# decadenza/SimpleStereo

Hardware: AMD Instinct MI355X
Metric: disparity MPixels/s (H*W*nDisp per second) (higher is better)
Workload: dtype f32

## Files before the change

### simplestereo_amd/csrc/asw_pipe_kernel.hip.h

```cpp
#pragma once
#include "asw_kernels.hip.h"
#ifndef SSAMD_KERNEL_TU
#include "lab_kernels.hip.h"
#endif

#ifndef SSAMD_PIPE_SENTINEL
#define SSAMD_PIPE_SENTINEL 1
#endif

namespace ssamd {

#ifndef SSAMD_KERNEL_TU
static constexpr int TADV_COLS = 64;
template <bool BYTES>
__device__ __forceinline__ void asw_tad_tile(const void *__restrict__ srcL, const void *__restrict__ srcR, unsigned char *__restrict__ evol,
                                             int W, int pad, int minD, int Dc, int Se, int erow0, int erows, int evolW, int rd, long long npix_total,
                                             int bx, int by, int bz, char *smem)
{
    uint32_t *const sL = reinterpret_cast<uint32_t *>(smem);
    uint32_t *const sR = sL + TADV_COLS;
    const int r = erow0 + by, z = bz, uc0 = bx * TADV_COLS;
    const int P = Se >> 2, dlo = minD + z * Dc, dhi = dlo + Dc - 1;
    const int u0 = uc0 - pad, xr0 = u0 - dhi;
    auto pixel = [&](const void *src, int col) -> uint32_t {
        const size_t q = (size_t)r * W + col;
        if constexpr (BYTES) {
            typedef uint32_t __attribute__((aligned(1))) u32_unaligned;
            const uint8_t *const b = reinterpret_cast<const uint8_t *>(src) + 3 * q;
            return (long long)q + 1 < npix_total ? (*reinterpret_cast<const u32_unaligned *>(b) & 0xffffffu)
                                                 : ((uint32_t)b[0] | ((uint32_t)b[1] << 8) | ((uint32_t)b[2] << 16));
        } else {
            return reinterpret_cast<const PixRec *>(src)[q].bgrx;
        }
    };
    for (int k = threadIdx.x; k < 2 * TADV_COLS + Dc; k += blockDim.x) {
        const bool isL = k < TADV_COLS;
        const int col = isL ? u0 + k : xr0 + (k - TADV_COLS);
        const uint32_t v = (unsigned)col < (unsigned)W ? pixel(isL ? srcL : srcR, col) : 0x80000000u;
        (isL ? sL : sR)[isL ? k : k - TADV_COLS] = v;
    }
    __syncthreads();
    const int ncols = min(TADV_COLS, evolW - uc0);
    uint32_t *const out = reinterpret_cast<uint32_t *>(evol + (((size_t)z * erows + by) * (size_t)evolW + uc0) * Se);
    auto dword = [&](int c, int slot, uint32_t lp) {
        uint32_t v = 0;
        const int d0 = rd == 6 ? 6 * (slot >> 1) + 4 * (slot & 1) : 4 * slot, nv = rd == 6 && (slot & 1) ? 2 : 4;
        if (!(lp >> 31) && d0 < Dc) {
            const uint32_t *const rp = sR + c + (Dc - 1) - d0;
#pragma unroll
            for (int q = 0; q < 4; ++q) {
                const uint32_t rv = q < nv && d0 + q < Dc ? rp[-q] : 0x80000000u;
                if (!(rv >> 31)) v |= min(__builtin_amdgcn_sad_u8(lp, rv, 0u), 40u) << (8 * q);
            }
        }
        return v;
    };
    if ((P & 3) == 0) {
        const int P4 = P >> 2;
        uint4 *const out4 = reinterpret_cast<uint4 *>(out);
        for (int k = threadIdx.x; k < ncols * P4; k += blockDim.x) {
            const int c = k / P4, s4 = 4 * (k - c * P4);
            const uint32_t lp = sL[c];
            out4[k] = make_uint4(dword(c, s4, lp), dword(c, s4 + 1, lp), dword(c, s4 + 2, lp), dword(c, s4 + 3, lp));
        }
        return;
    }
    for (int k = threadIdx.x; k < ncols * P; k += blockDim.x) {
        const int c = k / P, slot = k - c * P;
        out[k] = dword(c, slot, sL[c]);
    }
}

__global__ __launch_bounds__(256) void asw_tad_volume_kernel(const PixRec *__restrict__ recL, const PixRec *__restrict__ recR,
                                                             unsigned char *__restrict__ evol, int W, int pad, int minD, int Dc,
                                                             int Se, int erow0, int erows, int evolW, int rd = 4)
{
    extern __shared__ __attribute__((aligned(16))) char smem[];
    asw_tad_tile<false>(recL, recR, evol, W, pad, minD, Dc, Se, erow0, erows, evolW, rd, 0, blockIdx.x, blockIdx.y, blockIdx.z, smem);
}

struct AswPrepassArgs {
    const uint8_t *bgrL, *bgrR;
    PixRec *recL, *recR;
    unsigned char *evol;
    long long npix_total;
    int W, pad, minD, Dc, Se, erow0, erows, evolW, rd;
    int lab_blocks, ex, ey;
};
__global__ __launch_bounds__(256) void asw_prepass_kernel(const AswPrepassArgs P)
{
    extern __shared__ __attribute__((aligned(16))) char smem[];
    if ((int)blockIdx.x < P.lab_blocks) {
        SSAMD_LAB_TABLES_IN_LDS(T)
        const long long np = (long long)P.erows * P.W, first = (long long)P.erow0 * P.W;
        const uint8_t *const bl = P.bgrL + 3 * first, *const br = P.bgrR + 3 * first;
        PixRec *const rl = P.recL + first, *const rr = P.recR + first;
        typedef uint32_t __attribute__((aligned(1))) u32_unaligned;
        for (long long q = (long long)blockIdx.x * blockDim.x + threadIdx.x; q < 2 * np; q += (long long)P.lab_blocks * blockDim.x) {
            const bool right = q >= np;
            const long long p = right ? q - np : q;
            const uint8_t *const bgr = right ? br : bl;
            uint32_t B, G, R;
            if (p + 1 < np) {
                const uint32_t v = *reinterpret_cast<const u32_unaligned *>(bgr + 3 * p);
                B = v & 0xff; G = (v >> 8) & 0xff; R = (v >> 16) & 0xff;
            } else {
                B = bgr[3 * p]; G = bgr[3 * p + 1]; R = bgr[3 * p + 2];
            }
            PixRec o;
            bgr_to_lab(B, G, R, o.L, o.a, o.b, T);
            o.bgrx = B | (G << 8) | (R << 16);
            (right ? rr : rl)[p] = o;
        }
        return;
    }
    const int b = (int)blockIdx.x - P.lab_blocks, bx = b % P.ex, by = (b / P.ex) % P.ey, bz = b / (P.ex * P.ey);
    asw_tad_tile<true>(P.bgrL, P.bgrR, P.evol, P.W, P.pad, P.minD, P.Dc, P.Se, P.erow0, P.erows, P.evolW, P.rd, P.npix_total, bx, by, bz, smem);
}

#endif

template <bool WITH_COSTS, int SLC = 0, int SRC = 0, int SEC = 0, bool CG = false>
__global__ __launch_bounds__(ASW_MAX_THREADS, 3) void asw_aggregate_pipe_kernel(const AswArgs A)
{
    constexpr bool STATIC = SLC > 0;
    static_assert(!CG || STATIC, "compile-time geometry belongs to a static tile");
    constexpr int RX = ASW_RX;
    constexpr int NWR = asw_nwr(RX);
    extern __shared__ __attribute__((aligned(16))) char smem[];
    constexpr AswGeom SG = asw_pipe_geom_constexpr(AswPipeTile<SLC, SRC, SEC>::id);
    static_assert(!STATIC || (SG.SL == SLC && SG.SR == SRC && SG.Se == SEC), "the strides name the tile");
    const AswGeom &g = CG ? SG : A.g;
    float *const wL = reinterpret_cast<float *>(smem + g.off_wL);
    float *const wR = reinterpret_cast<float *>(smem + g.off_wR);
    unsigned char *const eT0 = reinterpret_cast<unsigned char *>(smem + g.off_e);
    float4 *const labL = reinterpret_cast<float4 *>(smem + g.off_labL);
    float4 *const labR = reinterpret_cast<float4 *>(smem + g.off_labR);
    uint32_t *const bgrL = reinterpret_cast<uint32_t *>(smem + g.off_bgrL);
    uint32_t *const bgrR = reinterpret_cast<uint32_t *>(smem + g.off_bgrR);
    u64 *const bestL = reinterpret_cast<u64 *>(smem + g.off_bestL);
    u64 *const bestR = reinterpret_cast<u64 *>(smem + g.off_bestR);
    float4 *const cenLab = reinterpret_cast<float4 *>(smem + g.off_cen);
    float *const proxS = reinterpret_cast<float *>(smem + g.off_prox);

    const int tid = threadIdx.x, nthr = blockDim.x;
    const int W = A.W, win = CG ? AswPipeTile<SLC, SRC, SEC>::id.win : A.win, p = CG ? AswPipeTile<SLC, SRC, SEC>::id.win / 2 : A.pad;
    const int Tx = g.Tx, Dc = g.Dc, nL = g.nL, nR = g.nR, nRc = g.nRc, SR = g.SR, Se = g.Se;
    const int JC = g.JC, NC = g.NC;
    int bx = blockIdx.x;
    if ((gridDim.x & 7) == 0) bx = (bx & 7) * (gridDim.x >> 3) + (bx >> 3);
    const int x0 = bx * Tx;
    const int y = asw_out_row(A, blockIdx.y);
    const int dlo = A.minD + blockIdx.z * Dc;
    const int dhi = dlo + Dc - 1;
    if (min(x0 + Tx - 1, W - 1) - dlo < 0) {
        if (A.disp)
            for (int k = threadIdx.x; k < Tx && x0 + k < W; k += blockDim.x)
                A.disp[(size_t)(y - A.row0) * W + x0 + k] = (int16_t)(x0 + k);
        return;
    }
    const int segL_lo = x0 - p, xrc_lo = x0 - dhi, segR_lo = xrc_lo - p;
    const int phase = g.dephase ? __builtin_amdgcn_readfirstlane((int)(threadIdx.x >> 8)) : 1;

    float accN[RX][ASW_RD], accS[RX][ASW_RD];
#pragma unroll
    for (int a = 0; a < RX; ++a)
#pragma unroll
        for (int b = 0; b < ASW_RD; ++b) { accN[a][b] = 0.f; accS[a][b] = 0.f; }

    for (int k = tid; k < Tx; k += nthr) bestL[k] = KEY_NONE;
    for (int k = tid; k <= nRc; k += nthr) bestR[k] = KEY_NONE;
    for (int c = tid; c < Tx + nRc; c += nthr) {
        const bool isL = c < Tx;
        const int ccol = isL ? x0 + c : xrc_lo + (c - Tx);
        float4 v = make_float4(0.f, 0.f, 0.f, 0.f);
        if ((unsigned)ccol < (unsigned)W) {
            const PixRec q = (isL ? A.recL : A.recR)[(size_t)y * W + ccol];
            v = make_float4(q.L, q.a, q.b, 1.f);
        }
        cenLab[c] = v;
    }

    const int i_lo = max(0, p - y), i_hi = min(win, A.H + p - y);

    auto stage_row = [&](int i) {
        int tids = threadIdx.x;
        asm volatile("" : "+v"(tids));
        const int buf = i & 1, r = y - p + i;
        for (int k = tids; k < win; k += nthr) proxS[buf * win + k] = A.prox[i * win + k];
        const PixRec *const rowL = A.recL + (size_t)r * W;
        const PixRec *const rowR = A.recR + (size_t)r * W;
        for (int k = tids; k < nL + nR; k += nthr) {
            const bool isL = k < nL;
            const int idx = isL ? k : k - nL;
            const int col = (isL ? segL_lo : segR_lo) + idx;
            PixRec v;
            v.L = SSAMD_PIPE_SENTINEL ? __builtin_inff() : 0.f;
            v.a = v.b = 0.f;
            v.bgrx = 0u;
            if ((unsigned)col < (unsigned)W) v = (isL ? rowL : rowR)[col];
            (isL ? labL + buf * nL : labR + buf * nR)[idx] = make_float4(v.L, v.a, v.b, 0.f);
            if (!A.evol) (isL ? bgrL + buf * nL : bgrR + buf * nR)[idx] = v.bgrx;
        }
    };
    auto build_e = [&](int i, int t_lo, int t_hi) {
        int tidb = threadIdx.x;
        asm volatile("" : "+v"(tidb));
        unsigned char *const eT = eT0 + (i & 1) * g.e_bytes;
        const uint32_t *const bgrLc = bgrL + (i & 1) * nL, *const bgrRc = bgrR + (i & 1) * nR;
        const int e_q = nthr / nL, e_r = nthr - e_q * nL;
        int t = t_lo + tidb;
        int sp = t / nL, ul = t - sp * nL;
        while (t < t_hi) {
            const uint32_t lp = bgrLc[ul];
            const uint32_t *const rp = bgrRc + (ul + (Dc - 1) - 8 * sp);
            uint32_t lo = 0, hi = 0;
#pragma unroll
            for (int k = 0; k < 4; ++k) {
                lo |= min(__builtin_amdgcn_sad_u8(lp, rp[-k], 0u), 40u) << (8 * k);
                hi |= min(__builtin_amdgcn_sad_u8(lp, rp[-4 - k], 0u), 40u) << (8 * k);
            }
            uint32_t *const dst = reinterpret_cast<uint32_t *>(eT + ul * Se) + 2 * sp;
            dst[0] = lo;
            if (2 * sp + 1 < g.DG) dst[1] = hi;
            t += nthr; ul += e_r; sp += e_q;
            if (ul >= nL) { ul -= nL; ++sp; }
        }
    };
    auto load_e = [&](int i) {
        int tidd = threadIdx.x;
        asm volatile("" : "+v"(tidd));
        const int r = y - p + i;
        const unsigned char *const src = A.evol + (((size_t)blockIdx.z * A.erows + (r - A.erow0)) * (size_t)A.evolW + x0) * Se;
        unsigned char *const dst = eT0 + (i & 1) * g.e_bytes;
        const int bytes = nL * Se, lane16 = (tidd & 63) * 16;
        for (int k = __builtin_amdgcn_readfirstlane(tidd >> 6) * 1024; k < bytes; k += (nthr >> 6) * 1024)
            if (k + lane16 < bytes)
                __builtin_amdgcn_global_load_lds((const void *)(src + k + lane16),
                                                 (__attribute__((address_space(3))) void *)(dst + k), 16, 0, 0);
    };
    auto build_weights = [&](int i, int jb, int je, int rb) {
        int tidw = threadIdx.x;
        asm volatile("" : "+v"(tidw));
        const float4 *const labLc = labL + (i & 1) * nL, *const labRc = labR + (i & 1) * nR;
        const float *const prow = proxS + (i & 1) * win;
        const int ncen = Tx + nRc;
        const int full = ncen / nthr * nthr, rest = ncen - full;
        int slen = je - jb, nseg = 1;
        if (rest > 0 && full > 0) {
            slen = max(ASW_WB, (je - jb + nthr / rest - 1) / (nthr / rest));
            slen = (slen + ASW_WB - 1) / ASW_WB * ASW_WB;
            nseg = (je - jb + slen - 1) / slen;
        }
        const int ntasks = full + rest * nseg;
        for (int t = tidw; t < ntasks; t += nthr) {
            int c = t, jb_t = jb, je_t = je;
            if (t >= full && nseg > 1) {
                const int q = t - full, sgm = q / rest;
                c = full + q - sgm * rest;
                jb_t = jb + sgm * slen;
                je_t = min(je, jb_t + slen);
            }
            const bool isL = c < Tx;
            const int cc = isL ? c : c - Tx;
            const float4 cen = cenLab[c];
            const float4 *const seg = (isL ? labLc : labRc) + cc;
            const int stride = isL ? g.SL : SR;
            float *const wout = (isL ? wL : wR) + cc + (rb - jb) * stride;
            const int col0 = (isL ? x0 : xrc_lo) + cc - p;
            const uint32_t cmask = cen.w != 0.f ? 0xffffffffu : 0u;
            int j = jb_t;
            const float4 *sp = seg + j;
            const float *pp = prow + j;
            float *wp = wout + j * stride;
            int col = col0 + j;
            const int stride4 = ASW_WB * stride;
            for (; j + ASW_WB <= je_t; j += ASW_WB, sp += ASW_WB, pp += ASW_WB, wp += stride4, col += ASW_WB) {
                float4 tp[ASW_WB];
                float pr[ASW_WB], wv[ASW_WB];
#pragma unroll
                for (int u = 0; u < ASW_WB; ++u) { tp[u] = sp[u]; pr[u] = pp[u]; }
#pragma unroll
                for (int u = 0; u < ASW_WB; ++u) {
                    asm volatile("" ::"v"(tp[u].w));
                    const float dL = tp[u].x - cen.x, da = tp[u].y - cen.y, db = tp[u].z - cen.z;
                    wv[u] = fmaf(db, db, fmaf(da, da, dL * dL));
                }
#pragma unroll
                for (int u = 0; u < ASW_WB; ++u) wv[u] = __builtin_amdgcn_sqrtf(wv[u]);
#pragma unroll
                for (int u = 0; u < ASW_WB; ++u) wv[u] = asw_weight_finish(wv[u], A.kC, pr[u]);
#pragma unroll
                for (int u = 0; u < ASW_WB; ++u) {
                    if constexpr (SSAMD_PIPE_SENTINEL) {
                        wp[u * stride] = wv[u];
                    } else {
                        const uint32_t m = (unsigned)(col + u) < (unsigned)W ? cmask : 0u;
                        wp[u * stride] = __uint_as_float(__float_as_uint(wv[u]) & m);
                    }
                }
            }
            if (j < je_t) {
                float4 tp[ASW_WB];
                float pr[ASW_WB], wv[ASW_WB];
#pragma unroll
                for (int u = 0; u < ASW_WB; ++u) {
                    const int jj = min(j + u, je_t - 1);
                    tp[u] = seg[jj];
                    pr[u] = prow[jj];
                }
#pragma unroll
                for (int u = 0; u < ASW_WB; ++u) {
                    asm volatile("" ::"v"(tp[u].w));
                    const float dL = tp[u].x - cen.x, da = tp[u].y - cen.y, db = tp[u].z - cen.z;
                    wv[u] = fmaf(db, db, fmaf(da, da, dL * dL));
                }
#pragma unroll
                for (int u = 0; u < ASW_WB; ++u) wv[u] = __builtin_amdgcn_sqrtf(wv[u]);
#pragma unroll
                for (int u = 0; u < ASW_WB; ++u) wv[u] = asw_weight_finish(wv[u], A.kC, pr[u]);
#pragma unroll
                for (int u = 0; u < ASW_WB; ++u) {
                    const int jj = min(j + u, je_t - 1);
                    if constexpr (SSAMD_PIPE_SENTINEL) {
                        wout[jj * stride] = wv[u];
                    } else {
                        const uint32_t m = (unsigned)(col0 + jj) < (unsigned)W ? cmask : 0u;
                        wout[jj * stride] = __uint_as_float(__float_as_uint(wv[u]) & m);
                    }
                }
            }
        }
    };
    auto chunk_end = [&](int c) { return c == NC - 1 ? win : (c + 1) * JC; };
    const int nE = nL * ((g.DG + 1) >> 1);
    auto build_next = [&](int i, int c, int cb) {
        const bool more_rows = i + 1 < i_hi;
#ifdef SSAMD_PIPE_BUILD_PRIO
        __builtin_amdgcn_s_setprio(SSAMD_PIPE_BUILD_PRIO);
#endif
#ifndef SSAMD_ABLATE_STAGE
        if (c == 0 && more_rows) stage_row(i + 1);
#endif
        if (c == 0 && more_rows && A.evol) load_e(i + 1);
#ifndef SSAMD_ABLATE_WEIGHTS
        if (c + 1 < NC) build_weights(i, (c + 1) * JC, chunk_end(c + 1), (cb ^ 1) * g.JCmax);
        else if (more_rows) build_weights(i + 1, 0, chunk_end(0), (cb ^ 1) * g.JCmax);
#endif
#ifndef SSAMD_ABLATE_E
        if (c >= 1 && more_rows && !A.evol) build_e(i + 1, (int)((long long)nE * (c - 1) / (NC - 1)), (int)((long long)nE * c / (NC - 1)));
#endif
#ifdef SSAMD_PIPE_BUILD_PRIO
        __builtin_amdgcn_s_setprio(0);
#endif
    };

    stage_row(i_lo);
    if (A.evol) load_e(i_lo);
    __syncthreads();
    if (!A.evol) build_e(i_lo, 0, nE);
    build_weights(i_lo, 0, chunk_end(0), 0);

    const int DGe = max(1, min(g.DG, (min(min(x0 + Tx, W) - 1, x0 + Tx - 1) - dlo) / ASW_RD + 1));
    const int nact = g.XG * DGe;
    int pk_xd;
    bool run;
    {
        const int tidm = threadIdx.x;
        int xg, dg;
#ifdef SSAMD_PIPE_PLAIN_LANES
        xg = tidm / DGe; dg = tidm - xg * DGe;
#else
        const int F = DGe >> 4, Lo = DGe & 15, nfull = g.XG * F;
        const int grp16 = tidm >> 4, r16 = tidm & 15;
        if (grp16 < nfull) {
            xg = grp16 / F;
            int gi = grp16 - xg * F;
            if (xg & 1) gi = F - 1 - gi;
            dg = 16 * gi + r16;
        } else {
            const int q = tidm - 16 * nfull;
            xg = Lo ? q / Lo : g.XG;
            dg = 16 * F + (Lo ? q - xg * Lo : 0);
        }
#endif
        pk_xd = xg | (dg << 16);
        const bool tile_live = tidm < nact && x0 + RX * xg < W && dlo + ASW_RD * dg <= A.maxD &&
                               x0 + RX * xg + RX - 1 - (dlo + ASW_RD * dg) >= 0;
        run = __builtin_amdgcn_ballot_w64(tile_live) != 0 && tidm < nact;
    }

    int cb = 0;
#pragma nounroll
    for (int i = i_lo; i < i_hi; ++i) {
        const unsigned char *const eT = eT0 + (i & 1) * g.e_bytes;
        AswRow ew[RX];

#pragma nounroll
        for (int c = 0; c < NC; ++c) {
#ifndef SSAMD_ABLATE_BARRIER
            __syncthreads();
#endif
            const int jc = c * JC, jend = chunk_end(c);
            const int rb = cb * g.JCmax;
            if (phase == 0) build_next(i, c, cb);
#ifndef SSAMD_ABLATE_AGG
            if (run) {
                const int xg = pk_xd & 0xffff, dg = pk_xd >> 16;
                const unsigned char *erow = eT + (RX * xg + (jc == 0 ? 0 : RX - 1 + jc)) * Se + 4 * dg;
                if (jc == 0) {
#pragma unroll
                    for (int n = 0; n < RX - 1; ++n) {
                        asw_row_unpack(ew[n], *reinterpret_cast<const uint32_t *>(erow));
                        erow += Se;
                    }
                }
                const float *wlp = wL + rb * g.SL + 8 * xg;
                const float *wrp = wR + rb * SR + (RX * xg - ASW_RD * dg + Dc - ASW_RD);
                for (int j0 = jc; j0 < jend; j0 += RX) {
#define SSAMD_PSTEP(JJ)                                                                             \
    if (j0 + (JJ) < jend) {                                                                         \
        const uint32_t epk = *reinterpret_cast<const uint32_t *>(erow + (STATIC ? (JJ) * SEC : 0)); \
        if constexpr (!STATIC) erow += Se;                                                          \
        float wl[RX], wr[NWR];                                                                      \
        {                                                                                           \
            const float *const wl_ = wlp + (STATIC ? (JJ) * SLC : 0);                              \
            const float *const wr_ = wrp + (STATIC ? (JJ) * SRC : 0);                              \
            const float4 v0 = *reinterpret_cast<const float4 *>(wl_);                              \
            wl[0] = v0.x; wl[1] = v0.y; wl[2] = v0.z; wl[3] = v0.w;                                 \
            const float4 v1 = *reinterpret_cast<const float4 *>(wl_ + 4);                          \
            wl[4] = v1.x; wl[5] = v1.y; wl[6] = v1.z; wl[7] = v1.w;                                 \
            const float4 r0 = *reinterpret_cast<const float4 *>(wr_);                              \
            const float4 r1 = *reinterpret_cast<const float4 *>(wr_ + 4);                          \
            const float4 r2 = *reinterpret_cast<const float4 *>(wr_ + 8);                          \
            asm volatile("" ::"v"(r2.w));       \
            wr[0] = r0.x; wr[1] = r0.y; wr[2] = r0.z; wr[3] = r0.w;                                 \
            wr[4] = r1.x; wr[5] = r1.y; wr[6] = r1.z; wr[7] = r1.w;                                 \
            wr[8] = r2.x; wr[9] = r2.y; wr[10] = r2.z; wr[11] = r2.w;                               \
        }                                                                                           \
        if constexpr (!STATIC) { wlp += g.SL; wrp += SR; }                                         \
               \
        _Pragma("unroll") for (int xi = 0; xi < RX; ++xi) {                                         \
            if (xi == RX - 1) asw_row_unpack(ew[((JJ) + RX - 1) % RX], epk);                        \
            const AswRow &row_ = ew[((JJ) + xi) % RX];                                              \
            _Pragma("unroll") for (int di = 0; di < ASW_RD; ++di) {                                 \
                const float w_ = wl[xi] * wr[xi - di + ASW_RD - 1];                                 \
                accN[xi][di] = fmaf(w_, row_.e[di], accN[xi][di]);                                  \
                accS[xi][di] = fmaf(w_, row_.c[di], accS[xi][di]);                                  \
            }                                                                                       \
        }                                                                                           \
    }
                    SSAMD_PSTEP(0) SSAMD_PSTEP(1) SSAMD_PSTEP(2) SSAMD_PSTEP(3)
                    SSAMD_PSTEP(4) SSAMD_PSTEP(5) SSAMD_PSTEP(6) SSAMD_PSTEP(7)
#undef SSAMD_PSTEP
                    if constexpr (STATIC) { erow += RX * SEC; wlp += RX * SLC; wrp += RX * SRC; }
                }
            }
#endif
            if (phase != 0) build_next(i, c, cb);
            cb ^= 1;
        }
    }

    int tidf = threadIdx.x;
    asm volatile("" : "+v"(tidf));
    AswKeyTile<RX, ASW_RD> kt;
    if (tidf < nact) {
        const int xg = pk_xd & 0xffff, dg = pk_xd >> 16;
        u64 diag[RX + ASW_RD - 1];
#pragma unroll
        for (int k = 0; k < RX + ASW_RD - 1; ++k) diag[k] = KEY_NONE;
#pragma unroll
        for (int xi = 0; xi < RX; ++xi) {
            const int x = x0 + RX * xg + xi;
            u64 bl = KEY_NONE;
#pragma unroll
            for (int di = 0; di < ASW_RD; ++di) {
                const int d = dlo + ASW_RD * dg + di;
                const bool valid = (x < W) && (d <= A.maxD) && (x - d >= 0);
                kt.v[xi][di] = 0xffffffffu;
                if (valid) {
                    float c;
                    const u64 hi = (u64)asw_cost_key(accN[xi][di], accS[xi][di], c) << 32;
                    kt.v[xi][di] = (uint32_t)(hi >> 32);
                    bl = min(bl, hi | (u64)(uint32_t)d);
                    diag[xi - di + ASW_RD - 1] = min(diag[xi - di + ASW_RD - 1], hi | (u64)(uint32_t)x);
                    if (WITH_COSTS)
                        A.costs[((size_t)(y - A.row0) * W + x) * (A.maxD - A.minD + 1) + (d - A.minD)] = A.cost_keys ? __uint_as_float((uint32_t)(hi >> 32)) : c;
                }
            }
            if (bl != KEY_NONE) atomicMin(&bestL[RX * xg + xi], bl);
        }
        if (A.keyR) {
            const int base = RX * xg - ASW_RD * dg + Dc - ASW_RD;
#pragma unroll
            for (int k = 0; k < RX + ASW_RD - 1; ++k)
                if (diag[k] != KEY_NONE) atomicMin(&bestR[base + k], diag[k]);
        }
    }
    __syncthreads();
    const size_t orow = (size_t)(y - A.row0) * W;
    const bool xq = !WITH_COSTS && A.xq.entries != nullptr;
    if (xq) {
        const int xg = pk_xd & 0xffff, dg = pk_xd >> 16;
        asw_exact_select<RX, ASW_RD>(A.xq, tidf < nact, kt, bestL + RX * xg, A.keyR ? bestR + (RX * xg - ASW_RD * dg + Dc - ASW_RD) : nullptr,
                                     x0 + RX * xg, dlo + ASW_RD * dg, (uint32_t)orow, exact_zkey(win));
    }
    if (A.disp) {
        for (int k = tid; k < Tx; k += nthr) {
            const int x = x0 + k;
            if (x < W) A.disp[orow + x] = bestL[k] == KEY_NONE ? (int16_t)x : (int16_t)(uint32_t)bestL[k];
        }
        return;
    }
    if (xq) {
        for (int k0 = 0; k0 < Tx; k0 += nthr) {
            const int k = k0 + tid, x = x0 + k;
            const bool have = k < Tx && x < W && bestL[k < Tx ? k : 0] != KEY_NONE;
            const u64 mine = have ? bestL[k] : KEY_NONE;
            const u64 old = have ? atomicMin(&A.keyL[orow + x], mine) : KEY_NONE;
            asw_exact_merge<false>(A.xq, have, mine, old, (uint32_t)orow, x, exact_zkey(win));
        }
        if (A.keyR)
            for (int k0 = 0; k0 < nRc; k0 += nthr) {
                const int k = k0 + tid, xr = xrc_lo + k;
                const bool have = k < nRc && (unsigned)xr < (unsigned)W && bestR[k < nRc ? k : 0] != KEY_NONE;
                const u64 mine = have ? bestR[k] : KEY_NONE;
                const u64 old = have ? atomicMin(&A.keyR[orow + xr], mine) : KEY_NONE;
                asw_exact_merge<true>(A.xq, have, mine, old, (uint32_t)orow, xr, exact_zkey(win));
            }
        return;
    }
    for (int k = tid; k < Tx; k += nthr) {
        const int x = x0 + k;
        if (x < W && bestL[k] != KEY_NONE) atomicMin(&A.keyL[orow + x], bestL[k]);
    }
    if (A.keyR) {
        for (int k = tid; k < nRc; k += nthr) {
            const int xr = xrc_lo + k;
            if ((unsigned)xr < (unsigned)W && bestR[k] != KEY_NONE) atomicMin(&A.keyR[orow + xr], bestR[k]);
        }
    }
}

}
```

Before: 10570.

## Stage Lab rows via global_load_lds DMA on dedicated waves, flatten weight tasks

Replaces the register round-trip row staging of Lab records and proximity weights with global_load_lds direct-to-LDS transfers, issued after the weight build and optionally restricted to waves beyond the first four when dephasing is on. The weight builder is reflattened into uniform (center, batch) tasks so the work splits evenly across threads instead of using the old segment-splitting heuristic. An explicit vmcnt(0) wait is added before each chunk barrier to make the asynchronous copies visible. Optional timestamp instrumentation is added behind a macro that is off by default.

```diff
diff --git a/simplestereo_amd/csrc/asw_pipe_kernel.hip.h b/simplestereo_amd/csrc/asw_pipe_kernel.hip.h
--- a/simplestereo_amd/csrc/asw_pipe_kernel.hip.h
+++ b/simplestereo_amd/csrc/asw_pipe_kernel.hip.h
@@ -8,7 +8,19 @@
 #define SSAMD_PIPE_SENTINEL 1
 #endif
 
+#ifndef SSAMD_PIPE_ROW_DMA
+#define SSAMD_PIPE_ROW_DMA 1
+#endif
+#ifndef SSAMD_PIPE_CEN_B128
+#define SSAMD_PIPE_CEN_B128 0
+#endif
+
 namespace ssamd {
+
+#ifdef SSAMD_PIPE_STAMPS
+static constexpr int PIPE_STAMP_WAVES = 12, PIPE_STAMP_ROWS = 64, PIPE_STAMP_CHUNKS = 4, PIPE_STAMP_KINDS = 5;
+__device__ unsigned long long pipe_stamps[PIPE_STAMP_WAVES * PIPE_STAMP_ROWS * PIPE_STAMP_CHUNKS * PIPE_STAMP_KINDS];
+#endif
 
 #ifndef SSAMD_KERNEL_TU
 static constexpr int TADV_COLS = 64;
@@ -182,6 +194,18 @@
     }
 
     const int i_lo = max(0, p - y), i_hi = min(win, A.H + p - y);
+#ifdef SSAMD_PIPE_STAMPS
+    const bool stamp_on = blockIdx.x == gridDim.x / 2 && blockIdx.y == gridDim.y / 2 && blockIdx.z == 0 && NC <= PIPE_STAMP_CHUNKS &&
+                          nthr <= 64 * PIPE_STAMP_WAVES && win <= PIPE_STAMP_ROWS;
+#define SSAMD_STAMP(I, C, KIND)                                                                                              \
+    if (stamp_on) {                                                                                                          \
+        const unsigned long long t_ = __builtin_amdgcn_s_memtime();                                                          \
+        if ((threadIdx.x & 63) == 0)                                                                                         \
+            pipe_stamps[(((threadIdx.x >> 6) * PIPE_STAMP_ROWS + (I)) * PIPE_STAMP_CHUNKS + (C)) * PIPE_STAMP_KINDS + (KIND)] = t_; \
+    }
+#else
+#define SSAMD_STAMP(I, C, KIND)
+#endif
 
     auto stage_row = [&](int i) {
         int tids = threadIdx.x;
@@ -227,122 +251,124 @@
             if (ul >= nL) { ul -= nL; ++sp; }
         }
     };
-    auto load_e = [&](int i) {
+    auto load_e = [&](int i, int w0) {
         int tidd = threadIdx.x;
         asm volatile("" : "+v"(tidd));
         const int r = y - p + i;
         const unsigned char *const src = A.evol + (((size_t)blockIdx.z * A.erows + (r - A.erow0)) * (size_t)A.evolW + x0) * Se;
         unsigned char *const dst = eT0 + (i & 1) * g.e_bytes;
         const int bytes = nL * Se, lane16 = (tidd & 63) * 16;
-        for (int k = __builtin_amdgcn_readfirstlane(tidd >> 6) * 1024; k < bytes; k += (nthr >> 6) * 1024)
+        for (int k = (__builtin_amdgcn_readfirstlane(tidd >> 6) - w0) * 1024; k < bytes; k += ((nthr >> 6) - w0) * 1024)
             if (k + lane16 < bytes)
                 __builtin_amdgcn_global_load_lds((const void *)(src + k + lane16),
                                                  (__attribute__((address_space(3))) void *)(dst + k), 16, 0, 0);
     };
+    auto stage_row_dma = [&](int i, int w0) {
+        int tids = threadIdx.x;
+        asm volatile("" : "+v"(tids));
+        const int buf = i & 1, r = y - p + i, lane = tids & 63;
+        const PixRec *const rowL = A.recL + (size_t)r * W;
+        const PixRec *const rowR = A.recR + (size_t)r * W;
+        const int pL = (nL + 63) >> 6, pR = (nR + 63) >> 6, pP = (win + 63) >> 6;
+        for (int q = __builtin_amdgcn_readfirstlane(tids >> 6) - w0; q < pL + pR + pP; q += (nthr >> 6) - w0) {
+            if (q < pL + pR) {
+                const bool isL = q < pL;
+                const int k = (isL ? q : q - pL) << 6, idx = k + lane;
+                const int col = (isL ? segL_lo : segR_lo) + idx;
+                float4 *const dst = (isL ? labL + buf * nL : labR + buf * nR) + k;
+                if (idx < (isL ? nL : nR)) {
+                    if ((unsigned)col < (unsigned)W)
+                        __builtin_amdgcn_global_load_lds((const void *)((isL ? rowL : rowR) + col),
+                                                         (__attribute__((address_space(3))) void *)dst, 16, 0, 0);
+                    else {
+                        float sl = SSAMD_PIPE_SENTINEL ? __builtin_inff() : 0.f, sz = 0.f;
+                        asm volatile("" : "+v"(sl), "+v"(sz));
+                        dst[lane] = make_float4(sl, sz, sz, sz);
+                    }
+                }
+            } else {
+                const int k = (q - pL - pR) << 6;
+                if (k + lane < win)
+                    __builtin_amdgcn_global_load_lds((const void *)(A.prox + i * win + k + lane),
+                                                     (__attribute__((address_space(3))) void *)(proxS + buf * win + k), 4, 0, 0);
+            }
+        }
+    };
+    auto weight_batch = [&](int i, int c, int j, int je_t, int jb, int rb) {
+        const float4 *const labLc = labL + (i & 1) * nL, *const labRc = labR + (i & 1) * nR;
+        const float *const prow = proxS + (i & 1) * win;
+        const bool isL = c < Tx;
+        const int cc = isL ? c : c - Tx;
+        const float4 cen = cenLab[c];
+#if SSAMD_PIPE_CEN_B128
+        asm volatile("" ::"v"(cen.w));
+#endif
+        const float4 *const seg = (isL ? labLc : labRc) + cc;
+        const int stride = isL ? g.SL : SR;
+        float *const wout = (isL ? wL : wR) + cc + (rb - jb) * stride;
+        const int col0 = (isL ? x0 : xrc_lo) + cc - p;
+        const uint32_t cmask = cen.w != 0.f ? 0xffffffffu : 0u;
+        float4 tp[ASW_WB];
+        float pr[ASW_WB], wv[ASW_WB];
+        const bool whole = j + ASW_WB <= je_t;
+        if (whole) {
+#pragma unroll
+            for (int u = 0; u < ASW_WB; ++u) { tp[u] = seg[j + u]; pr[u] = prow[j + u]; }
+        } else {
+#pragma unroll
+            for (int u = 0; u < ASW_WB; ++u) {
+                const int jj = min(j + u, je_t - 1);
+                tp[u] = seg[jj];
+                pr[u] = prow[jj];
+            }
+        }
+#pragma unroll
+        for (int u = 0; u < ASW_WB; ++u) {
+            asm volatile("" ::"v"(tp[u].w));
+            const float dL = tp[u].x - cen.x, da = tp[u].y - cen.y, db = tp[u].z - cen.z;
+            wv[u] = fmaf(db, db, fmaf(da, da, dL * dL));
+        }
+#pragma unroll
+        for (int u = 0; u < ASW_WB; ++u) wv[u] = __builtin_amdgcn_sqrtf(wv[u]);
+#pragma unroll
+        for (int u = 0; u < ASW_WB; ++u) wv[u] = asw_weight_finish(wv[u], A.kC, pr[u]);
+#pragma unroll
+        for (int u = 0; u < ASW_WB; ++u) {
+            const int jj = whole ? j + u : min(j + u, je_t - 1);
+            if constexpr (SSAMD_PIPE_SENTINEL) {
+                wout[jj * stride] = wv[u];
+            } else {
+                const uint32_t m = (unsigned)(col0 + jj) < (unsigned)W ? cmask : 0u;
+                wout[jj * stride] = __uint_as_float(__float_as_uint(wv[u]) & m);
+            }
+        }
+    };
     auto build_weights = [&](int i, int jb, int je, int rb) {
         int tidw = threadIdx.x;
         asm volatile("" : "+v"(tidw));
-        const float4 *const labLc = labL + (i & 1) * nL, *const labRc = labR + (i & 1) * nR;
-        const float *const prow = proxS + (i & 1) * win;
         const int ncen = Tx + nRc;
-        const int full = ncen / nthr * nthr, rest = ncen - full;
-        int slen = je - jb, nseg = 1;
-        if (rest > 0 && full > 0) {
-            slen = max(ASW_WB, (je - jb + nthr / rest - 1) / (nthr / rest));
-            slen = (slen + ASW_WB - 1) / ASW_WB * ASW_WB;
-            nseg = (je - jb + slen - 1) / slen;
-        }
-        const int ntasks = full + rest * nseg;
+        const int nbat = (je - jb + ASW_WB - 1) / ASW_WB, ntasks = ncen * nbat;
+        const int dq = nthr / ncen, dr = nthr - dq * ncen;
+        int b = tidw / ncen, c = tidw - b * ncen;
         for (int t = tidw; t < ntasks; t += nthr) {
-            int c = t, jb_t = jb, je_t = je;
-            if (t >= full && nseg > 1) {
-                const int q = t - full, sgm = q / rest;
-                c = full + q - sgm * rest;
-                jb_t = jb + sgm * slen;
-                je_t = min(je, jb_t + slen);
-            }
-            const bool isL = c < Tx;
-            const int cc = isL ? c : c - Tx;
-            const float4 cen = cenLab[c];
-            const float4 *const seg = (isL ? labLc : labRc) + cc;
-            const int stride = isL ? g.SL : SR;
-            float *const wout = (isL ? wL : wR) + cc + (rb - jb) * stride;
-            const int col0 = (isL ? x0 : xrc_lo) + cc - p;
-            const uint32_t cmask = cen.w != 0.f ? 0xffffffffu : 0u;
-            int j = jb_t;
-            const float4 *sp = seg + j;
-            const float *pp = prow + j;
-            float *wp = wout + j * stride;
-            int col = col0 + j;
-            const int stride4 = ASW_WB * stride;
-            for (; j + ASW_WB <= je_t; j += ASW_WB, sp += ASW_WB, pp += ASW_WB, wp += stride4, col += ASW_WB) {
-                float4 tp[ASW_WB];
-                float pr[ASW_WB], wv[ASW_WB];
-#pragma unroll
-                for (int u = 0; u < ASW_WB; ++u) { tp[u] = sp[u]; pr[u] = pp[u]; }
-#pragma unroll
-                for (int u = 0; u < ASW_WB; ++u) {
-                    asm volatile("" ::"v"(tp[u].w));
-                    const float dL = tp[u].x - cen.x, da = tp[u].y - cen.y, db = tp[u].z - cen.z;
-                    wv[u] = fmaf(db, db, fmaf(da, da, dL * dL));
-                }
-#pragma unroll
-                for (int u = 0; u < ASW_WB; ++u) wv[u] = __builtin_amdgcn_sqrtf(wv[u]);
-#pragma unroll
-                for (int u = 0; u < ASW_WB; ++u) wv[u] = asw_weight_finish(wv[u], A.kC, pr[u]);
-#pragma unroll
-                for (int u = 0; u < ASW_WB; ++u) {
-                    if constexpr (SSAMD_PIPE_SENTINEL) {
-                        wp[u * stride] = wv[u];
-                    } else {
-                        const uint32_t m = (unsigned)(col + u) < (unsigned)W ? cmask : 0u;
-                        wp[u * stride] = __uint_as_float(__float_as_uint(wv[u]) & m);
-                    }
-                }
-            }
-            if (j < je_t) {
-                float4 tp[ASW_WB];
-                float pr[ASW_WB], wv[ASW_WB];
-#pragma unroll
-                for (int u = 0; u < ASW_WB; ++u) {
-                    const int jj = min(j + u, je_t - 1);
-                    tp[u] = seg[jj];
-                    pr[u] = prow[jj];
-                }
-#pragma unroll
-                for (int u = 0; u < ASW_WB; ++u) {
-                    asm volatile("" ::"v"(tp[u].w));
-                    const float dL = tp[u].x - cen.x, da = tp[u].y - cen.y, db = tp[u].z - cen.z;
-                    wv[u] = fmaf(db, db, fmaf(da, da, dL * dL));
-                }
-#pragma unroll
-                for (int u = 0; u < ASW_WB; ++u) wv[u] = __builtin_amdgcn_sqrtf(wv[u]);
-#pragma unroll
-                for (int u = 0; u < ASW_WB; ++u) wv[u] = asw_weight_finish(wv[u], A.kC, pr[u]);
-#pragma unroll
-                for (int u = 0; u < ASW_WB; ++u) {
-                    const int jj = min(j + u, je_t - 1);
-                    if constexpr (SSAMD_PIPE_SENTINEL) {
-                        wout[jj * stride] = wv[u];
-                    } else {
-                        const uint32_t m = (unsigned)(col0 + jj) < (unsigned)W ? cmask : 0u;
-                        wout[jj * stride] = __uint_as_float(__float_as_uint(wv[u]) & m);
-                    }
-                }
-            }
+            weight_batch(i, c, jb + b * ASW_WB, je, jb, rb);
+            c += dr; b += dq;
+            if (c >= ncen) { c -= ncen; ++b; }
         }
     };
     auto chunk_end = [&](int c) { return c == NC - 1 ? win : (c + 1) * JC; };
     const int nE = nL * ((g.DG + 1) >> 1);
     auto build_next = [&](int i, int c, int cb) {
         const bool more_rows = i + 1 < i_hi;
+        SSAMD_STAMP(i - i_lo, c, 1)
 #ifdef SSAMD_PIPE_BUILD_PRIO
         __builtin_amdgcn_s_setprio(SSAMD_PIPE_BUILD_PRIO);
 #endif
+        const bool row_dma = SSAMD_PIPE_ROW_DMA && A.evol;
 #ifndef SSAMD_ABLATE_STAGE
-        if (c == 0 && more_rows) stage_row(i + 1);
-#endif
-        if (c == 0 && more_rows && A.evol) load_e(i + 1);
+        if (c == 0 && more_rows && !row_dma) stage_row(i + 1);
+#endif
+        if (c == 0 && more_rows && A.evol && !row_dma) load_e(i + 1, 0);
 #ifndef SSAMD_ABLATE_WEIGHTS
         if (c + 1 < NC) build_weights(i, (c + 1) * JC, chunk_end(c + 1), (cb ^ 1) * g.JCmax);
         else if (more_rows) build_weights(i + 1, 0, chunk_end(0), (cb ^ 1) * g.JCmax);
@@ -350,13 +376,26 @@
 #ifndef SSAMD_ABLATE_E
         if (c >= 1 && more_rows && !A.evol) build_e(i + 1, (int)((long long)nE * (c - 1) / (NC - 1)), (int)((long long)nE * c / (NC - 1)));
 #endif
+        if (c == 0 && more_rows && row_dma) {
+            int tidq = threadIdx.x;
+            asm volatile("" : "+v"(tidq));
+            const int w0 = g.dephase && (nthr >> 6) > 4 ? 4 : 0;
+            if (__builtin_amdgcn_readfirstlane(tidq >> 6) >= w0) {
+#ifndef SSAMD_ABLATE_STAGE
+                stage_row_dma(i + 1, w0);
+#endif
+                load_e(i + 1, w0);
+            }
+        }
 #ifdef SSAMD_PIPE_BUILD_PRIO
         __builtin_amdgcn_s_setprio(0);
 #endif
-    };
-
-    stage_row(i_lo);
-    if (A.evol) load_e(i_lo);
+        SSAMD_STAMP(i - i_lo, c, 2)
+    };
+
+    if (SSAMD_PIPE_ROW_DMA && A.evol) stage_row_dma(i_lo, 0);
+    else stage_row(i_lo);
+    if (A.evol) load_e(i_lo, 0);
     __syncthreads();
     if (!A.evol) build_e(i_lo, 0, nE);
     build_weights(i_lo, 0, chunk_end(0), 0);
@@ -398,9 +437,11 @@
 
 #pragma nounroll
         for (int c = 0; c < NC; ++c) {
+            asm volatile("s_waitcnt vmcnt(0)" ::: "memory");
 #ifndef SSAMD_ABLATE_BARRIER
             __syncthreads();
 #endif
+            SSAMD_STAMP(i - i_lo, c, 0)
             const int jc = c * JC, jend = chunk_end(c);
             const int rb = cb * g.JCmax;
             if (phase == 0) build_next(i, c, cb);
@@ -417,6 +458,7 @@
                 }
                 const float *wlp = wL + rb * g.SL + 8 * xg;
                 const float *wrp = wR + rb * SR + (RX * xg - ASW_RD * dg + Dc - ASW_RD);
+                SSAMD_STAMP(i - i_lo, c, 3)
                 for (int j0 = jc; j0 < jend; j0 += RX) {
 #define SSAMD_PSTEP(JJ)                                                                             \
     if (j0 + (JJ) < jend) {                                                                         \
@@ -458,10 +500,12 @@
             }
 #endif
             if (phase != 0) build_next(i, c, cb);
+            SSAMD_STAMP(i - i_lo, c, 4)
             cb ^= 1;
         }
     }
 
+#undef SSAMD_STAMP
     int tidf = threadIdx.x;
     asm volatile("" : "+v"(tidf));
     AswKeyTile<RX, ASW_RD> kt;
@@ -543,4 +587,12 @@
     }
 }
 
+#if defined(SSAMD_PIPE_STAMPS) && !defined(SSAMD_KERNEL_TU)
+extern "C" __attribute__((visibility("default"))) int ssamd_pipe_stamps_read(unsigned long long *dst, int n)
+{
+    if (n != (int)(sizeof(pipe_stamps) / sizeof(pipe_stamps[0]))) return -1;
+    return (int)hipMemcpyFromSymbol(dst, HIP_SYMBOL(pipe_stamps), sizeof(pipe_stamps));
 }
+#endif
+
+}
```

After: 9270. 0.877x the previous value.
